# JoeMWatson/input-inference-for-control

Measured on AMD Instinct MI355X. Metric: i2c timestep-messages/sec (cell-iterations/s = B*T*EM-iters/s), pendulum T=200 B=4096 per GPU, higher is better.
Workload: dtype f64; 1 GPU; pendulum_known_quad cubature i2c (nx=2, nu=1, nz=4), T=200, B=4096 trajectories per GPU, global batch 4096, CubatureQuadrature(1,0,0), alpha0=100, tol=0; batch_per_gpu=4096, horizon=200, parallelism=batch-sharded x1, no collective in the EM loop, kernels=one lane per trajectory

## Files before the change

input-inference-for-control_amd/csrc/i2c_cell.hpp:

```cpp
#pragma once
#include <stdint.h>
#include <type_traits>
#include "../../include/i2c_hip.h"
#include "i2c_linalg.hpp"
#include "i2c_models.hpp"

namespace i2c {

template <typename R> struct Rule {
  R sf;
  R w0;
  R wi;
  R W;
  int unit;
  int gh_degree, gh_points;
  R gh_x[I2C_MAX_GH_DEGREE], gh_w[I2C_MAX_GH_DEGREE];
};

template <class M> struct PerTraj : M {};
template <class M> struct is_per_traj : std::false_type {};
template <class M> struct is_per_traj<PerTraj<M>> : std::true_type {};
template <typename R, bool PER_TRAJ> struct ParamsB {};
template <typename R> struct ParamsB<R, true> {
  const R* params_b;
// ... 1354 lines not shown
    for (int i = 0; i < NX; ++i) r.m3f[i] = in[(long)(O_MU3 + i) * B];
#pragma unroll
    for (int i = 0; i < sym(NX); ++i) r.S3f[i] = in[(long)(O_S3 + i) * B];
#pragma unroll
    for (int i = 0; i < NX * NX; ++i) r.Jx[i] = in[(long)(O_J + i) * B];
  };
  Row cur, nxt;
  load(t_hi - 1, cur);
  for (int t = t_hi - 1; t >= t_lo; --t) {
    load(t > t_lo ? t - 1 : t_lo, nxt);
    const R* mu1 = cur.mu1;
    const R* S1 = cur.S1;
    const R* m3f = cur.m3f;
    const R* Jx = cur.Jx;
    R S3n[sym(NX)];
#pragma unroll
    for (int i = 0; i < sym(NX); ++i) S3n[i] = Cc[i] - cur.S3f[i];
    R an[NX], Gn[NX * NX];
#pragma unroll
    for (int i = 0; i < NX; ++i) {
      R v = mu1[i];
#pragma unroll
      for (int k = 0; k < NX; ++k) v += Jx[i * NX + k] * (av[k] - m3f[k]);
      an[i] = v;
    }
#pragma unroll
    for (int i = 0; i < sym(NX); ++i) Cc[i] = S1[i];
    add_JDJt<NX, NX>(Jx, S3n, Cc);
#pragma unroll
    for (int i = 0; i < NX; ++i)
#pragma unroll
      for (int j = 0; j < NX; ++j) {
        R v = R(0);
#pragma unroll
        for (int k = 0; k < NX; ++k) v += Jx[i * NX + k] * G[k * NX + j];
        Gn[i * NX + j] = v;
      }
#pragma unroll
    for (int i = 0; i < NX; ++i) av[i] = an[i];
#pragma unroll
    for (int i = 0; i < NX * NX; ++i) G[i] = Gn[i];
    cur = nxt;
  }
  constexpr int EC = NX + NX * NX + sym(NX);
  R* out = a.comp + ((long)ch * EC) * B + b;
#pragma unroll
  for (int i = 0; i < NX; ++i) out[(long)i * B] = av[i];
#pragma unroll
  for (int i = 0; i < NX * NX; ++i) out[(long)(NX + i) * B] = G[i];
#pragma unroll
  for (int i = 0; i < sym(NX); ++i) out[(long)(NX + NX * NX + i) * B] = Cc[i];
}

template <class M, typename R, typename S_ = R, int GRID = 0>
I2C_HD inline void chunk_stitch_body(const Consts<M, R>& c, const ChunkArgs<R, S_>& a, const int b) {
  using C = Consts<M, R>;
  constexpr int NX = C::NX, D = C::D;
  constexpr int O_MU3 = D + sym(D), O_S3 = O_MU3 + NX, EC = NX + NX * NX + sym(NX);
  const long B = c.B;
  const S_* last = a.cell.fwd + ((long)(c.T - 1) * C::E_FWD) * B + b;
  R m3f[NX], S3f[sym(NX)], m[NX], S[sym(NX)];
#pragma unroll
  for (int i = 0; i < NX; ++i) m3f[i] = last[(long)(O_MU3 + i) * B];
#pragma unroll
  for (int i = 0; i < sym(NX); ++i) S3f[i] = last[(long)(O_S3 + i) * B];
  end_of_chain<M, R>(c, a.cell.temp, b, m3f, S3f, m, S, a.cell.status);
  terminal_obs_stats<M, R, GRID>(c, b, m, S, a.cell.term_stats, a.cell.status);
  R av[NX], G[NX * NX], Cc[sym(NX)], nav[NX], nG[NX * NX], nCc[sym(NX)];
  auto loadc = [&](int ch, R* la, R* lG, R* lC) {
    const R* cp = a.comp + ((long)(ch > 0 ? ch : 0) * EC) * B + b;
#pragma unroll
    for (int i = 0; i < NX; ++i) la[i] = cp[(long)i * B];
#pragma unroll
    for (int i = 0; i < NX * NX; ++i) lG[i] = cp[(long)(NX + i) * B];
#pragma unroll
    for (int i = 0; i < sym(NX); ++i) lC[i] = cp[(long)(NX + NX * NX + i) * B];
  };
  loadc(a.n_chunks - 1, av, G, Cc);
  for (int ch = a.n_chunks - 1; ch >= 0; --ch) {
    loadc(ch - 1, nav, nG, nCc);
    R* bo = a.bnd + ((long)ch * C::E_XM) * B + b;
#pragma unroll
    for (int i = 0; i < NX; ++i) bo[(long)i * B] = m[i];
#pragma unroll
    for (int i = 0; i < sym(NX); ++i) bo[(long)(NX + i) * B] = S[i];
    R mn[NX];
#pragma unroll
    for (int i = 0; i < NX; ++i) {
      R v = av[i];
#pragma unroll
      for (int k = 0; k < NX; ++k) v += G[i * NX + k] * m[k];
      mn[i] = v;
    }
    add_JDJt<NX, NX>(G, S, Cc);
#pragma unroll
    for (int i = 0; i < NX; ++i) m[i] = mn[i];
#pragma unroll
    for (int i = 0; i < sym(NX); ++i) S[i] = Cc[i];
#pragma unroll
    for (int i = 0; i < NX; ++i) av[i] = nav[i];
#pragma unroll
    for (int i = 0; i < NX * NX; ++i) G[i] = nG[i];
#pragma unroll
    for (int i = 0; i < sym(NX); ++i) Cc[i] = nCc[i];
  }
}

template <class M, typename R, typename S_ = R, bool LEANW = false, int GRID = 0>
I2C_HD inline void chunk_walk_body(const Consts<M, R>& c, const ChunkArgs<R, S_>& a, const int ch, const int b) {
  using C = Consts<M, R>;
  constexpr int NX = C::NX, NZ = C::NZ, D = C::D;
  constexpr int O_MU3 = D + sym(D), O_S3 = O_MU3 + NX, O_J = O_S3 + sym(NX);
  constexpr unsigned W = sizeof(S_);
  const unsigned long B = c.B;
  const unsigned bo = (unsigned)b * W, rb = (unsigned)(B * W);
  const int t_lo = ch * a.chunk_len, t_hi = (t_lo + a.chunk_len < c.T) ? t_lo + a.chunk_len : c.T;
  CellArgs<R, S_> ca = a.cell;
  if (LEANW) ca.xm = nullptr, ca.zpost = nullptr, ca.cell_stats = nullptr;
  const bool z_per_cell = LEANW ? false : c.z_per_cell != 0;
  R m3m[NX], S3m[sym(NX)];
  {
    const R* bi = a.bnd + ((long)ch * C::E_XM) * B + b;
#pragma unroll
    for (int i = 0; i < NX; ++i) m3m[i] = bi[(long)i * B];
#pragma unroll
    for (int i = 0; i < sym(NX); ++i) S3m[i] = bi[(long)(NX + i) * B];
  }
  constexpr bool DOUBLE_BUFFER = C::D <= 5;
  constexpr bool VOFF = I2C_WALK_VOFF && C::D <= 5;
  constexpr int NOFF = C::E_FWD > C::E_POST ? (C::E_FWD > C::E_ZPOST ? C::E_FWD : C::E_ZPOST) : (C::E_POST > C::E_ZPOST ? C::E_POST : C::E_ZPOST);
  unsigned voff[VOFF ? NOFF : 1];
  if (VOFF) {
#pragma unroll
    for (int e = 0; e < NOFF; ++e) voff[e] = bo + (unsigned)e * rb;
  }
  PolyTab<R> ptab;
  if (VOFF) poly_tab_init(ptab);
  const PolyTab<R>* const tab = VOFF ? &ptab : nullptr;
  R row[C::E_FWD], nxt[DOUBLE_BUFFER ? C::E_FWD : 1];
  if (DOUBLE_BUFFER) {
    const Window w = make_window(ca.fwd + (unsigned long)(t_hi - 1) * C::E_FWD * B, (unsigned long)C::E_FWD * rb);
#pragma unroll
    for (int e = 0; e < C::E_FWD; ++e) row[e] = (R)wld<S_>(w, VOFF ? 0u : e * rb, VOFF ? voff[e] : bo);
    if (LEANW) {
#pragma unroll
      for (int e = 0; e < C::E_FWD; ++e) row[e] = opaque(row[e]);
    }
  }
  R sum_m = R(0), sum_v = R(0);
  for (int t = t_hi - 1; t >= t_lo; --t) {
    {
      const int tp = DOUBLE_BUFFER ? (t > t_lo ? t - 1 : t_lo) : t;
      const Window w = make_window(ca.fwd + (unsigned long)tp * C::E_FWD * B, (unsigned long)C::E_FWD * rb);
#pragma unroll
      for (int e = 0; e < C::E_FWD; ++e)
        (DOUBLE_BUFFER ? nxt[DOUBLE_BUFFER ? e : 0] : row[e]) = (R)wld<S_>(w, VOFF ? 0u : e * rb, VOFF ? voff[e] : bo);
    }
    if (ca.xm) {
      S_* xo = const_cast<S_*>(ca.xm) + ((long)t * C::E_XM) * B + b;
#pragma unroll
      for (int i = 0; i < NX; ++i) xo[(long)i * B] = (S_)m3m[i];
#pragma unroll
      for (int i = 0; i < sym(NX); ++i) xo[(long)(NX + i) * B] = (S_)S3m[i];
    }
    R dm[NX], dS[sym(NX)], zt[NZ];
#pragma unroll
    for (int i = 0; i < NX; ++i) dm[i] = m3m[i] - row[O_MU3 + i];
#pragma unroll
    for (int i = 0; i < sym(NX); ++i) dS[i] = S3m[i] - row[O_S3 + i];
    if (VOFF && z_per_cell) {
      static_assert(NZ <= NOFF, "row offsets");
      const Window wz = make_window(ca.z + (unsigned long)c.row(t) * NZ * B, (unsigned long)NZ * B * sizeof(R));
#pragma unroll
      for (int k = 0; k < NZ; ++k) zt[k] = wld<R>(wz, 0u, voff[k] * (unsigned)(sizeof(R) / W));
    } else {
#pragma unroll
      for (int k = 0; k < NZ; ++k) zt[k] = z_per_cell ? ca.z[((long)c.row(t) * NZ + k) * B + b] : c.zg[k];
    }
    R* mu = row;
    R* S = row + D;
    R ctl[C::E_POST - D - sym(D)], mz[NZ], Sz[sym(NZ)], cm, cv;
    if (!cell_posterior<M, R, GRID>(c, b, zt, mu, S, row + O_J, dm, dS, ctl, mz, Sz, &cm, &cv, tab)) set_status(ca.status, b, 7, t);
    store_cell<M, R, S_>(c, ca, t, b, mu, S, ctl, mz, Sz, cm, cv, VOFF ? voff : nullptr);
    sum_m += cm;
    sum_v += cv;
#pragma unroll
    for (int i = 0; i < NX; ++i) m3m[i] = mu[i];
#pragma unroll
    for (int i = 0; i < sym(NX); ++i) S3m[i] = S[i];
    if (DOUBLE_BUFFER) {
#pragma unroll
      for (int e = 0; e < C::E_FWD; ++e) row[e] = nxt[DOUBLE_BUFFER ? e : 0];
    }
  }
  a.part[((long)ch * 2 + 0) * B + b] = sum_m;
  a.part[((long)ch * 2 + 1) * B + b] = sum_v;
}

template <typename R> struct MstepArgs {
  const R* term_stats;
  R* alpha;
  R* stats_out;
  int update;
};

template <class M, typename R>
I2C_HD inline void mstep_body(const Consts<M, R>& c, const MstepArgs<R>& a, const int b) {
  using C = Consts<M, R>;
  const long B = c.B;
  const R stat = a.term_stats[B + b], v = a.term_stats[2 * B + b];
  const R m = c.inference == I2C_INF_LINEARIZE ? a.term_stats[(long)(C::E_TERM - 1) * B + b] : stat;
  R tr = stat, sf = R(C::NZ) * R(c.T);
  if (C::NZT > 0 && c.has_Qf) {
    tr += a.term_stats[b];
    sf += R(C::NZT);
  }
  const R alpha_hat = tr / sf;
  const R alpha = a.alpha[b];
  R alpha_new = alpha;
  if (a.update) {
    if (c.tol >= R(0)) {
      const R ratio = alpha_hat / alpha;
      alpha_new = alpha_hat;
      if (ratio < c.tol) alpha_new = c.tol * alpha;
      if (ratio > R(2) - c.tol) alpha_new = (R(2) - c.tol) * alpha;
    }
    a.alpha[b] = alpha_new;
  }
  a.stats_out[b] = alpha_hat;
  a.stats_out[B + b] = alpha_new;
  a.stats_out[2 * B + b] = m;
  a.stats_out[3 * B + b] = v;
}

template <typename R> struct PropArgs {
  const R* post;
  R* prop;
  R* prop_stats;
  const R* x0;
  const R* sig_x0;
  const R* z;
  const uint8_t* ff;
  int32_t* status;
  const uint8_t* expert;
};

template <class M, typename R, int GRID = 0>
I2C_HD inline void propagate_body(const Consts<M, R>& c, const PropArgs<R>& a, const int b) {
  using C = Consts<M, R>;
  constexpr int NX = C::NX, NU = C::NU, NZ = C::NZ, D = C::D;
  const long B = c.B;
  const int T = c.T;
  const bool wr = grid_writer<GRID>();
  R mu_x[NX], sig_x[sym(NX)];
#pragma unroll
  for (int i = 0; i < NX; ++i) mu_x[i] = a.x0[i * B + b];
#pragma unroll
  for (int i = 0; i < sym(NX); ++i) sig_x[i] = a.sig_x0[i * B + b];
  constexpr bool PREFETCH = C::D <= 5;
  R pri[C::E_PRI];
  if (PREFETCH) {
#pragma unroll
    for (int e = 0; e < C::E_PRI; ++e) pri[e] = a.post[((long)c.row(0) * C::E_POST + e) * B + b];
  }
  unsigned ff_cur = a.ff[c.row(0)], ex_cur = a.expert ? (unsigned)a.expert[c.row(0)] : (unsigned)(c.use_expert != 0);
  ff_cur = opaque(ff_cur);
  ex_cur = opaque(ex_cur);
  if (PREFETCH) {
#pragma unroll
    for (int e = 0; e < C::E_PRI; ++e) pri[e] = opaque(pri[e]);
  }
#pragma unroll
  for (int i = 0; i < NX; ++i) mu_x[i] = opaque(mu_x[i]);
#pragma unroll
  for (int i = 0; i < sym(NX); ++i) sig_x[i] = opaque(sig_x[i]);
  constexpr bool ZPRE = PREFETCH && NZ <= NX * 4;
  R zt_cur[ZPRE ? NZ : 1];
  auto fetch_z = [&](const int row, R* zt) {
    const R* src = c.z_per_cell ? a.z + ((long)row * NZ) * B + b : a.x0 + b;
    const long st = c.z_per_cell ? B : 0;
#pragma unroll
    for (int k = 0; k < NZ; ++k) {
      const R v = src[(long)k * st];
      zt[k] = c.z_per_cell ? v : c.zg[k];
    }
// ... 446 lines not shown
```

input-inference-for-control_amd/csrc/i2c_impl.hpp:

```cpp
#pragma once
#include "i2c_entry.hpp"
#include "i2c_cell.hpp"
#include "i2c_group.hpp"
#include "i2c_wave.hpp"
#include "i2c_quad.hpp"
#include "i2c_grid.hpp"
#include "i2c_linearize.hpp"

#include <cmath>
#include <cstdlib>
#include <cstring>

namespace i2c {

constexpr int SWEEP_BLOCK = 64;
#ifndef I2C_LANE_BLOCK
#define I2C_LANE_BLOCK 64
#endif
constexpr int LANE_BLOCK = I2C_LANE_BLOCK;
constexpr int CELL_BLOCK = 256;

#ifdef I2C_HOST_SIM
#define I2C_KERNEL(BLOCK) static void
#define I2C_LANE_PARAMS const long lane_x_, const int lane_y_,
// ... 31 lines not shown
  return hipMemcpyAsync(dst, src, n, hipMemcpyDeviceToDevice, (hipStream_t)stream) == hipSuccess ? I2C_OK : I2C_ELAUNCH;
}
#endif

template <class M, typename R, bool LEAN, bool GRID = false, typename S = R>
I2C_KERNEL(LANE_BLOCK) k_forward(I2C_LANE_PARAMS const Consts<M, R> c, const FwdArgs<R, S> a, const int block) {
  const long b = I2C_LANE_X(block);
  if (b < c.B) forward_sweep_body<M, R, LEAN, GRID, S>(c, a, (int)b);
}
template <class M, typename R> I2C_KERNEL(LANE_BLOCK) k_forward_lin(I2C_LANE_PARAMS const Consts<M, R> c, const FwdArgs<R> a) {
  const long b = I2C_LANE_X(LANE_BLOCK);
  if (b < c.B) forward_lin_body<M, R>(c, a, (int)b);
}
template <class M, typename R> I2C_KERNEL(LANE_BLOCK) k_bwd_lin(I2C_LANE_PARAMS const Consts<M, R> c, const CellArgs<R> a) {
  const long b = I2C_LANE_X(LANE_BLOCK);
  if (b < c.B) backward_lin_body<M, R>(c, a, (int)b);
}
template <class M, typename R> I2C_KERNEL(LANE_BLOCK) k_riccati(I2C_LANE_PARAMS const Consts<M, R> c, const RiccatiArgs<R> a) {
  const long b = I2C_LANE_X(LANE_BLOCK);
  if (b < c.B) riccati_body<M, R>(c, a, (int)b);
}
template <class M, typename R, typename S = R>
I2C_KERNEL(LANE_BLOCK) k_scan(I2C_LANE_PARAMS const Consts<M, R> c, const ScanArgs<R, S> a) {
  const long b = I2C_LANE_X(LANE_BLOCK);
  if (b < c.B) backward_scan_body<M, R, S>(c, a, (int)b);
}
template <class M, typename R, typename S = R>
I2C_KERNEL(CELL_BLOCK) k_cell(I2C_LANE_PARAMS const Consts<M, R> c, const CellArgs<R, S> a) {
  const long b = I2C_LANE_X(CELL_BLOCK);
  if (b < c.B) backward_cell_body<M, R, S>(c, a, I2C_LANE_Y, (int)b);
}
template <class M, typename R, bool GRID = false, typename S = R, bool LEANW = false>
I2C_KERNEL(LANE_BLOCK) k_bwd_fused(I2C_LANE_PARAMS const Consts<M, R> c, const CellArgs<R, S> a) {
  const long b = I2C_LANE_X(LANE_BLOCK);
  if (b < c.B) backward_fused_body<M, R, GRID, S, LEANW>(c, a, (int)b);
}
template <class M, typename R, typename S = R>
I2C_KERNEL(LANE_BLOCK) k_chunk_compose(I2C_LANE_PARAMS const Consts<M, R> c, const ChunkArgs<R, S> a) {
  const long b = I2C_LANE_X(LANE_BLOCK);
  if (b < c.B) chunk_compose_body<M, R, S>(c, a, I2C_LANE_Y, (int)b);
}
template <class M, typename R, typename S = R, bool GRID = false>
I2C_KERNEL(LANE_BLOCK) k_chunk_stitch(I2C_LANE_PARAMS const Consts<M, R> c, const ChunkArgs<R, S> a) {
  const long b = I2C_LANE_X(LANE_BLOCK);
  if (b < c.B) chunk_stitch_body<M, R, S, GRID>(c, a, (int)b);
}
#ifndef I2C_WALK_LEAN
#define I2C_WALK_LEAN 1
#endif
template <class M, typename R, typename S = R, bool LEANW = false, bool GRID = false>
I2C_KERNEL(LANE_BLOCK) k_chunk_walk(I2C_LANE_PARAMS const Consts<M, R> c, const ChunkArgs<R, S> a) {
  const long b = I2C_LANE_X(LANE_BLOCK);
  if (b < c.B) chunk_walk_body<M, R, S, LEANW, GRID>(c, a, I2C_LANE_Y, (int)b);
}
template <class M, typename R> I2C_KERNEL(LANE_BLOCK) k_chunk_stitch_lin(I2C_LANE_PARAMS const Consts<M, R> c, const ChunkArgs<R, R> a) {
  const long b = I2C_LANE_X(LANE_BLOCK);
  if (b < c.B) chunk_stitch_lin_body<M, R>(c, a, (int)b);
}
template <class M, typename R> I2C_KERNEL(LANE_BLOCK) k_chunk_walk_lin(I2C_LANE_PARAMS const Consts<M, R> c, const ChunkArgs<R, R> a) {
  const long b = I2C_LANE_X(LANE_BLOCK);
  if (b < c.B) chunk_walk_lin_body<M, R>(c, a, I2C_LANE_Y, (int)b);
}
template <class M, typename R>
I2C_KERNEL(LANE_BLOCK) k_chunk_reduce_lin(I2C_LANE_PARAMS const Consts<M, R> c, const ChunkArgs<R, R> a, const MstepArgs<R> ms) {
  const long b = I2C_LANE_X(LANE_BLOCK);
  if (b < c.B) chunk_reduce_lin_body<M, R>(c, a, ms, (int)b);
}
template <class M, typename R> I2C_KERNEL(LANE_BLOCK) k_mstep(I2C_LANE_PARAMS const Consts<M, R> c, const MstepArgs<R> a) {
  const long b = I2C_LANE_X(LANE_BLOCK);
  if (b < c.B) mstep_body<M, R>(c, a, (int)b);
}
template <class M, typename R, bool GRID = false>
I2C_KERNEL(LANE_BLOCK) k_propagate(I2C_LANE_PARAMS const Consts<M, R> c, const PropArgs<R> a) {
  const long b = I2C_LANE_X(LANE_BLOCK);
  if (b < c.B) propagate_body<M, R, GRID>(c, a, (int)b);
}
template <class M, typename R, bool LEAN>
I2C_KERNEL(LANE_BLOCK) k_forward_propagate(I2C_LANE_PARAMS const Consts<M, R> c, const FwdArgs<R, R> af, const PropArgs<R> ap) {
  const long b = I2C_LANE_X(LANE_BLOCK);
  if (b >= c.B) return;
  if (I2C_LANE_Y == 0) forward_sweep_body<M, R, LEAN, false, R>(c, af, (int)b);
  else propagate_body<M, R, false>(c, ap, (int)b);
}
template <class M, typename R> struct ZetaArg {
  R v[sym(M::NY)];
};
template <class M, typename R>
I2C_KERNEL(LANE_BLOCK) k_ckf(I2C_LANE_PARAMS const Consts<M, R> c, const ZetaArg<M, R> z, const CkfArgs<R> a) {
  const long b = I2C_LANE_X(LANE_BLOCK);
  if (b < c.B) ckf_filter_body<M, R>(c, z.v, a, (int)b);
}
template <class M, typename R> I2C_KERNEL(CELL_BLOCK) k_mpc_shift(I2C_LANE_PARAMS const Consts<M, R> c, const ShiftArgs<R> a) {
  const long b = I2C_LANE_X(CELL_BLOCK);
  if (b < c.B) mpc_shift_body<M, R>(c, a, (int)b);
}
template <class M> I2C_KERNEL(CELL_BLOCK) k_to_feedback(I2C_LANE_PARAMS uint8_t* ff, const int t0, const int n, const int T) {
  const long i = I2C_LANE_X(CELL_BLOCK);
  if (i < n) ff[(t0 + (int)i) % T] = 0;
}
template <class M, typename R> I2C_KERNEL(LANE_BLOCK) k_rollout(I2C_LANE_PARAMS const Consts<M, R> c, const RolloutArgs<R> a) {
  const long n = I2C_LANE_X(LANE_BLOCK);
  if (n < (long)a.n_rollouts * c.B) rollout_body<M, R>(c, a, (int)n);
}
template <class M, typename R>
I2C_KERNEL(LANE_BLOCK) k_plant_step(I2C_LANE_PARAMS const Consts<M, R> c, const PlantNoise<M, R> nz, const PlantArgs<R> a) {
  const long b = I2C_LANE_X(LANE_BLOCK);
// ... 6 lines not shown
                          const R m, const R v) {
  a.term_stats[(long)c.B + b] = m;
  a.term_stats[2 * (long)c.B + b] = v;
  if (ms.alpha) {
    Consts<M, R> cm = c;
    cm.T = T_mstep;
    mstep_body<M, R>(cm, ms, b);
  }
}
#ifdef I2C_HOST_SIM
template <class M, typename R, class CA>
static int launch_reduce(const Consts<M, R>& c, const CA& a, const MstepArgs<R>& ms, const int T_mstep, void*) {
  for (int b = 0; b < c.B; ++b) {
    R m = R(0), v = R(0);
    for (int q = 0; q < REDUCE_PARTS; ++q) {
      R pm, pv;
      reduce_partial<M, R>(c, a.cell_stats, b, q, REDUCE_PARTS, &pm, &pv);
      m += pm;
      v += pv;
    }
    reduce_finish<M, R>(c, a, ms, T_mstep, b, m, v);
  }
  return I2C_OK;
}
#else
template <class M, typename R, class CA>
__global__ __launch_bounds__(SWEEP_BLOCK* REDUCE_PARTS) void k_reduce(const Consts<M, R> c, const CA a,
                                                                      const MstepArgs<R> ms, const int T_mstep) {
  __shared__ R sm[REDUCE_PARTS][SWEEP_BLOCK], sv[REDUCE_PARTS][SWEEP_BLOCK];
  const int b = blockIdx.x * SWEEP_BLOCK + threadIdx.x;
  R m = R(0), v = R(0);
  if (b < c.B) reduce_partial<M, R>(c, a.cell_stats, b, threadIdx.y, REDUCE_PARTS, &m, &v);
  sm[threadIdx.y][threadIdx.x] = m;
  sv[threadIdx.y][threadIdx.x] = v;
  __syncthreads();
  if (threadIdx.y == 0 && b < c.B) {
    m = sm[0][threadIdx.x];
    v = sv[0][threadIdx.x];
#pragma unroll
    for (int q = 1; q < REDUCE_PARTS; ++q) {
      m += sm[q][threadIdx.x];
      v += sv[q][threadIdx.x];
    }
    reduce_finish<M, R>(c, a, ms, T_mstep, b, m, v);
  }
}
template <class M, typename R, class CA>
static int launch_reduce(const Consts<M, R>& c, const CA& a, const MstepArgs<R>& ms, const int T_mstep, void* stream) {
  hipLaunchKernelGGL((k_reduce<M, R, CA>), dim3((c.B + SWEEP_BLOCK - 1) / SWEEP_BLOCK), dim3(SWEEP_BLOCK, REDUCE_PARTS), 0,
                     (hipStream_t)stream, c, a, ms, T_mstep);
  return hipGetLastError() == hipSuccess ? I2C_OK : I2C_ELAUNCH;
}
#endif


template <typename R> static bool unit_rule(const Rule<R>& r) { return r.unit && r.w0 == R(0); }
template <class M, typename R> static bool unit_rule(const Consts<M, R>& c) { return unit_rule(c.rule_xu) && unit_rule(c.rule_x); }

#ifdef I2C_HOST_SIM
template <typename R, class Body>
static void sim_teams(const int team, const long n_teams, const int n_rows, const bool rows_on_team, const size_t lds, const Body& body) {
  for (int y0 = 0; y0 < (rows_on_team ? 1 : n_rows); ++y0)
    for (long i = 0; i < n_teams; ++i) {
      std::vector<R> sh(lds, R(0)), xch(128, R(0));
      HostBarrier bar(team);
      std::vector<std::thread> lanes;
      for (int l = 0; l < team; ++l)
        lanes.emplace_back([&, l] {
          for (int y = y0; y < (rows_on_team ? n_rows : y0 + 1); ++y) body(i, y, l, lds ? sh.data() : (R*)nullptr, &bar, xch.data());
        });
      for (auto& th : lanes) th.join();
    }
}
#else
template <class M, typename R> __device__ __forceinline__ const Consts<M, R>* kernarg_consts() {
  return (const Consts<M, R>*)__builtin_amdgcn_kernarg_segment_ptr();
}
template <class M, typename R> __device__ __forceinline__ const R* kernarg_zeta() {
  constexpr size_t zoff = (sizeof(Consts<M, R>) + alignof(ZetaArg<M, R>) - 1) / alignof(ZetaArg<M, R>) * alignof(ZetaArg<M, R>);
  return ((const ZetaArg<M, R>*)((const char*)__builtin_amdgcn_kernarg_segment_ptr() + zoff))->v;
}
__device__ __forceinline__ long xcd_first_traj(const unsigned i) {
  const unsigned x = i & 7u, r = (i >> 3) & 3u, g = i >> 5;
  return 16L * (g * 8u + x) + 4 * r;
}
static unsigned xcd_blocks(const long B) { return (unsigned)((B + 127) / 128) * 32u; }
#endif

enum { GK_FORWARD = 0, GK_BACKWARD = 1, GK_PROPAGATE = 2, GK_CKF = 3 };
template <int KIND, class M, typename R, int G, bool FULLW, class KC, class A>
I2C_FN void group_body(const Consts<M, R>& c, const KC& kc, const A& a, const int b, const Grp<R, G>& g) {
  if constexpr (KIND == GK_FORWARD) forward_group_body<M, R, G, FULLW>(c, kc, a, b, g);
  if constexpr (KIND == GK_BACKWARD) backward_group_body<M, R, G, FULLW>(c, kc, a, b, g);
  if constexpr (KIND == GK_PROPAGATE) propagate_group_body<M, R, G, FULLW>(c, kc, a, b, g);
  if constexpr (KIND == GK_CKF) ckf_group_body<M, R, G>(c, kc, a, b, g);
}
#ifndef I2C_HOST_SIM
template <int KIND, class M, typename R, int G, bool FULLW, class A>
__global__ __launch_bounds__(SWEEP_BLOCK) void k_group(const Consts<M, R> c, const ZetaArg<M, R> zeta, const int has_zeta, const A a) {
  __shared__ GConst<M, R> kc;
  __shared__ R sh[(SWEEP_BLOCK / G) * Grp<R, G>::SIZE];
  gconst_fill<M, R>(kc, kernarg_consts<M, R>(), has_zeta ? kernarg_zeta<M, R>() : (const R*)nullptr, (int)threadIdx.x, SWEEP_BLOCK);
  __syncthreads();
  const long lane = (long)blockIdx.x * SWEEP_BLOCK + threadIdx.x;
  const long b = lane / G;
  if (b >= c.B) return;
// ... 383 lines not shown
  C c;
  std::memset(&c, 0, sizeof(c));
  c.B = p->B;
  c.T = p->T;
  c.t0 = p->t0;
  c.has_Qf = p->has_Qf && M::NZT > 0;
  c.has_x_terminal = p->has_x_terminal;
  c.z_per_cell = p->z_per_cell && p->z != nullptr;
  c.use_expert = use_expert;
  c.terminal_cell = p->terminal_cell;
  c.inference = p->inference;
  c.post_tm = (p->post_layout == 1 && M::WAVE) ? 1 : 0;
  auto is_diag = [](const double* W, int n) {
    for (int i = 0; i < n; ++i)
      for (int j = 0; j < i; ++j)
        if (W[i * (i + 1) / 2 + j] != 0.0) return 0;
    return 1;
  };
  c.qr_diag = is_diag(p->QR, C::NZ);
  c.qf_diag = is_diag(p->Qf, C::NZT);
  c.rule_xu = make_rule<R>(p, C::D);
  c.rule_x = make_rule<R>(p, C::NX);
  c.dtemp = (R)p->dtemp;
  c.tol = (R)tol;
  for (int i = 0; i < sym(C::NX); ++i) c.sig_eta[i] = (R)p->sig_eta[i];
  for (int i = 0; i < sym(C::NX); ++i) c.sig_eta_w[i] = c.rule_xu.W * c.sig_eta[i];
  for (int i = 0; i < sym(C::NZ); ++i) c.sig_xi0[i] = (R)p->sig_xi0[i];
  for (int i = 0; i < sym(C::NZ); ++i) c.QR[i] = (R)p->QR[i];
  for (int i = 0; i < sym(C::NZT); ++i) c.sig_xiT0[i] = (R)p->sig_xiT0[i];
  for (int i = 0; i < sym(C::NZT); ++i) c.Qf[i] = (R)p->Qf[i];
  for (int i = 0; i < C::NZ; ++i) c.zg[i] = (R)p->zg[i];
  for (int i = 0; i < C::NZT; ++i) c.zg_term[i] = (R)p->zg_term[i];
  for (int i = 0; i < C::NX; ++i) c.mu_x_term[i] = (R)p->mu_x_term[i];
  for (int i = 0; i < sym(C::NX); ++i) c.sig_x_term[i] = (R)p->sig_x_term[i];
  for (int i = 0; i < M::NP; ++i) c.params[i] = (R)p->model_params[i];
  if constexpr (is_per_traj<M>::value) c.params_b = (const R*)p->model_params_b;
  return c;
}

static void chunk_geometry(int B, int T, int* n_chunks, int* chunk_len) {
  static const int forced = [] {
    const char* e = getenv("I2C_CHUNKS");
    return e ? atoi(e) : 0;
  }();
  int nc = (65536 + B - 1) / B;
  if (nc > 32) nc = 32;
  if (nc > T / 4) nc = T / 4;
  if (forced > 0) nc = forced < T ? forced : T;
  if (nc < 1) nc = 1;
  const int len = (T + nc - 1) / nc;
  *chunk_len = len;
  *n_chunks = (T + len - 1) / len;
}
template <class M> struct ChunkWork {
  size_t bnd, part, total;
  ChunkWork(const int B, const int n_chunks) {
    constexpr int NX = M::NX;
    const size_t n = (size_t)n_chunks * (size_t)B;
    bnd = n * (NX + NX * NX + sym(NX));
    part = bnd + n * (NX + sym(NX));
    total = part + n * 3;
  }
};
template <class M> static size_t workspace_elems(int B, int T) {
  int nc, len;
  chunk_geometry(B, T, &nc, &len);
  return ChunkWork<M>(B, nc).total;
}
template <class M, typename R, typename S> static ChunkArgs<R, S> chunk_args(const I2cProblem* p, const CellArgs<R, S>& a) {
  ChunkArgs<R, S> ch{a, (R*)p->work, nullptr, nullptr, 0, 0};
  chunk_geometry(p->B, p->T, &ch.n_chunks, &ch.chunk_len);
  const ChunkWork<M> w(p->B, ch.n_chunks);
  ch.bnd = ch.comp + w.bnd;
  ch.part = ch.comp + w.part;
  return ch;
}

#define I2C_MODEL_CONST(name, MEMBER, DEFAULT)                                                                      \
  template <class M, class = void> struct name : std::integral_constant<int, (DEFAULT)> {};                         \
  template <class M> struct name<M, std::void_t<decltype(M::MEMBER)>> : std::integral_constant<int, M::MEMBER> {};
I2C_MODEL_CONST(bwd_fused_min_b, BWD_FUSED_MIN_B, I2C_BWD_FUSED_MIN_B)
I2C_MODEL_CONST(quad_backward_min_b, QUAD_BACKWARD8_MIN_B, 0)
I2C_MODEL_CONST(quad_backward_max_b, QUAD_BACKWARD8_MAX_B, -1)
I2C_MODEL_CONST(quad_chunk_walk_min_b, QUAD_CHUNK_WALK_MIN_B, 0)
I2C_MODEL_CONST(quad_chunk_walk_max_b, QUAD_CHUNK_WALK_MAX_B, -1)
I2C_MODEL_CONST(quad_chunk_passes_min_b, QUAD_CHUNK_PASSES_MIN_B, 0)
I2C_MODEL_CONST(quad_chunk_passes_max_b, QUAD_CHUNK_PASSES_MAX_B, -1)
I2C_MODEL_CONST(quad_chunk_stitch_max_b, QUAD_CHUNK_STITCH_MAX_B, -1)
#undef I2C_MODEL_CONST


struct Plan {
  int forward, backward, propagate, filter;
  int schedule;
  int walker;
  int compose, stitch;
  int rule;
  bool fwd_tm;
  bool fusable;
};

template <class M, typename R, typename S = R> struct Impl {
  using C = Consts<M, R>;
  static constexpr bool MIXED = sizeof(S) != sizeof(R);
  static constexpr int G = M::GROUP;
  static constexpr bool HAS_GROUP = G > 0 && sizeof(R) == 8 && !MIXED;
// ... 197 lines not shown

  static Plan resolve(const I2cProblem* p) {
    const Rule<R> rule_xu = make_rule<R>(p, C::D), rule_x = make_rule<R>(p, C::NX);
    const bool unit_xu = unit_rule(rule_xu), unit = unit_xu && unit_rule(rule_x);
    const Request req = request(p->group_lanes, p->inference);
    Plan pl;
    pl.rule = p->inference;
    pl.forward = forward_family(p, req, unit);
    pl.backward = backward_family(p, req, unit);
    pl.propagate = propagate_family(p, req, unit_xu || p->inference == I2C_INF_LINEARIZE);
    pl.filter = filter_family(p, req == REQ_GRID ? request(p->group_lanes, I2C_INF_CUBATURE) : req);
    pl.schedule = backward_schedule(p, req, pl.backward);
    const bool chunked = pl.schedule == I2C_BWD_CHUNKED;
    pl.walker = chunked ? pl.backward : I2C_ENOTSUP;
    pl.compose = pl.stitch = pl.schedule < 0 ? pl.schedule : I2C_ENOTSUP;
    if (chunked && p->inference == I2C_INF_CUBATURE) {
      pl.compose = quad_compose(p, req, unit) ? I2C_FAMILY_QUAD : I2C_FAMILY_LANE;
      pl.stitch = (pl.compose == I2C_FAMILY_QUAD || quad_stitch_alone(p, req, unit)) ? I2C_FAMILY_QUAD : I2C_FAMILY_LANE;
    }
    pl.fwd_tm = !MIXED && pl.forward == I2C_FAMILY_QUAD && ((M::WAVE && pl.backward == I2C_FAMILY_WAVE) || (HAS_QUAD_BACKWARD && pl.backward == I2C_FAMILY_QUAD));
    pl.fusable = LANE && C::D <= 5 && p->inference == I2C_INF_CUBATURE && pl.forward == I2C_FAMILY_LANE && pl.propagate == I2C_FAMILY_LANE &&
                 rule_xu.unit && rule_x.unit && !(p->z_per_cell && p->z) && !p->alpha_cell && p->t0 == 0;
    return pl;
  }
  static int plan(const I2cProblem* p) { return resolve(p).schedule; }
  static int family_of(const I2cProblem* p, const int sweep) {
    const Plan pl = resolve(p);
    const int of_sweep[] = {pl.forward, pl.backward, pl.propagate, pl.filter, pl.compose, pl.stitch};
    return of_sweep[sweep];
  }
  static int schedule_with(const Plan& pl, const bool workspace) {
    if (pl.schedule != I2C_BWD_CHUNKED || workspace) return pl.schedule;
    return (pl.rule == I2C_INF_CUBATURE && pl.walker != I2C_FAMILY_QUAD) ? I2C_BWD_TWO_PASS : I2C_BWD_FUSED;
  }

  static I2cProblem with_unit_rule(const I2cProblem* p) {
    I2cProblem q = *p;
    q.quad_alpha = 1.0, q.quad_beta = 0.0, q.quad_kappa = 0.0;
    return q;
  }
  static C forward_consts(const I2cProblem* p) { return make_consts<M, R>(p, 0.0, p->inference == I2C_INF_LINEARIZE ? p->expert_controller : 0); }
  static C propagate_consts(const I2cProblem* p, const int use_expert) {
    if (p->inference != I2C_INF_LINEARIZE) return make_consts<M, R>(p, 0.0, use_expert);
    const I2cProblem q = with_unit_rule(p);
    return make_consts<M, R>(&q, 0.0, use_expert);
  }
  static C filter_consts(const I2cProblem* p) {
    I2cProblem q = with_unit_rule(p);
    q.inference = I2C_INF_CUBATURE;
    return make_consts<M, R>(&q, 0.0, 0);
  }

  static int run_forward(const I2cProblem* p, const Plan& pl, const C& c, const void* prior, void* fwd, void* prior_out, int32_t* status,
                         void* stream) {
    if (pl.forward < 0) return pl.forward;
    const FwdArgs<R, S> a{(const S*)prior, (S*)fwd, (S*)prior_out, (const R*)p->x0, (const R*)p->sig_x0,
                          (const R*)p->z,  (const R*)p->alpha, (const R*)p->alpha_cell, p->feedforward, status, p->expert};
    if (pl.forward == I2C_FAMILY_WAVE) {
      if constexpr (HAS_WAVE) return launch_wave<WK_FORWARD, M, R, S>(c, a, stream);
    }
    if (pl.forward == I2C_FAMILY_QUAD) {
      if constexpr (HAS_QUAD) {
        C cq = c;
        cq.fwd_tm = pl.fwd_tm;
        return launch_quad_forward<M, R, S>(cq, a, stream);
      }
    }
    if (pl.forward == I2C_FAMILY_GROUP) {
      if constexpr (HAS_GROUP) return launch_group<GK_FORWARD, M, R, G>(c, nullptr, a, stream);
    }
    if (pl.forward == I2C_FAMILY_GRID) {
      if constexpr (HAS_GRID) return launch_grid<GRK_FORWARD, M, R>(c, a, stream);
    }
    if constexpr (LANE) {
      if constexpr (!MIXED) {
        if (pl.rule == I2C_INF_LINEARIZE) return launch(k_forward_lin<M, R>, p->B, 1, LANE_BLOCK, stream, c, a);
        if (pl.rule == I2C_INF_GAUSS_HERMITE) return launch(k_forward<M, R, false, true>, p->B, 1, LANE_BLOCK, stream, c, a, LANE_BLOCK);
      }
#ifdef I2C_HOST_SIM
      const int lanes = LANE_BLOCK;
#else
      const int lanes = sweep_lanes();
#endif
      const bool lean = c.rule_xu.unit && c.rule_x.unit && !c.z_per_cell && !a.alpha_cell && !a.prior_out && c.t0 == 0;
      if (lean) return launch(k_forward<M, R, true, false, S>, p->B, 1, lanes, stream, c, a, lanes);
      return launch(k_forward<M, R, false, false, S>, p->B, 1, lanes, stream, c, a, lanes);
    }
    return I2C_ENOTSUP;
  }
  static int forward(const I2cProblem* p, const void* prior, void* fwd, void* prior_out, int32_t* status, void* stream) {
    return run_forward(p, resolve(p), forward_consts(p), prior, fwd, prior_out, status, stream);
  }

  struct MstepFuse {
    double tol;
    int update;
    void* stats_out;
    bool done;
  };
  static const R* terminal_alpha(const I2cProblem* p, const C& c) {
    return p->alpha_cell ? (const R*)p->alpha_cell + (long)c.row(p->T - 1) * (long)p->B : (const R*)p->alpha;
  }
  static int run_backward(const I2cProblem* p, const Plan& pl, const C& c, const void* fwd, void* xm, void* post, void* zpost, void* cell_stats,
                          void* term_stats, int32_t* status, void* stream, MstepFuse* fuse) {
    if (pl.backward < 0) return pl.backward;
    if (pl.schedule < 0) return pl.schedule;
    const MstepArgs<R> ms{(const R*)term_stats, fuse ? (R*)p->alpha : nullptr, fuse ? (R*)fuse->stats_out : nullptr, fuse ? fuse->update : 0};
    const CellArgs<R, S> a{(const S*)fwd,  (const S*)xm,   (const R*)p->z, (S*)post, (S*)zpost,
                           (R*)cell_stats, (R*)term_stats, (R*)p->temp,    status,   terminal_alpha(p, c)};
    const int mode = schedule_with(pl, p->work != nullptr);
    int rc = I2C_ENOTSUP;
    if (pl.backward == I2C_FAMILY_WAVE) {
      if constexpr (HAS_WAVE) {
        if (mode != I2C_BWD_TWO_PASS || !a.xm || !a.cell_stats) return launch_wave<WK_BACKWARD, M, R, S>(c, a, stream);
        rc = launch_wave<WK_SCAN, M, R, S>(c, a, stream);
        if (rc == I2C_OK) rc = launch_wave<WK_CELL, M, R, S>(c, a, stream);
        if (rc == I2C_OK) rc = launch_reduce<M, R>(c, a, ms, p->T, stream);
        if (fuse) fuse->done = true;
      }
      return rc;
    }
    if (pl.backward == I2C_FAMILY_QUAD) {
      if constexpr (HAS_QUAD_BACKWARD) {
        if constexpr (QUAD8) {
          if (mode == I2C_BWD_CHUNKED) return backward_chunked(p, pl, c, a, ms, fuse, stream);
        }
        return launch_quad_backward<M, R, S>(c, a, stream);
      }
    }
    if (pl.backward == I2C_FAMILY_GROUP) {
      if constexpr (HAS_GROUP) return launch_group<GK_BACKWARD, M, R, G>(c, nullptr, a, stream);
    }
    if (pl.backward == I2C_FAMILY_GRID) {
      if constexpr (HAS_GRID) return launch_grid<GRK_BACKWARD, M, R>(c, a, stream);
    }
    if constexpr (LANE) {
      if (mode == I2C_BWD_CHUNKED) return backward_chunked(p, pl, c, a, ms, fuse, stream);
      if (mode == I2C_BWD_FUSED) {
        if constexpr (!MIXED) {
          if (pl.rule == I2C_INF_LINEARIZE) return launch(k_bwd_lin<M, R>, p->B, 1, LANE_BLOCK, stream, c, a);
          if (pl.rule == I2C_INF_GAUSS_HERMITE) return launch(k_bwd_fused<M, R, true>, p->B, 1, LANE_BLOCK, stream, c, a);
        }
        const bool lean = I2C_WALK_LEAN && !a.xm && !a.zpost && !a.cell_stats && !c.z_per_cell;
        return lean ? launch(k_bwd_fused<M, R, false, S, true>, p->B, 1, LANE_BLOCK, stream, c, a)
                    : launch(k_bwd_fused<M, R, false, S>, p->B, 1, LANE_BLOCK, stream, c, a);
      }
      if (!a.xm || !a.cell_stats) return I2C_EINVAL;
      const ScanArgs<R, S> sc{a.fwd, const_cast<S*>(a.xm), (R*)p->temp, a.status};
      rc = launch(k_scan<M, R, S>, p->B, 1, LANE_BLOCK, stream, c, sc);
      if (rc == I2C_OK) rc = launch(k_cell<M, R, S>, p->B, p->T, CELL_BLOCK, stream, c, a);
      if (rc == I2C_OK) rc = launch_reduce<M, R>(c, a, ms, p->T, stream);
      if (fuse) fuse->done = true;
    }
    return rc;
  }
  static int backward_chunked(const I2cProblem* p, const Plan& pl, const C& c, const CellArgs<R, S>& a, const MstepArgs<R>& ms, MstepFuse* fuse,
                              void* stream) {
    int rc = I2C_ENOTSUP;
    if constexpr (LANE) {
      const ChunkArgs<R, S> ch = chunk_args<M>(p, a);
      const long B = p->B;
      const int nc = ch.n_chunks;
      const bool lin = !MIXED && pl.rule == I2C_INF_LINEARIZE, gh = !MIXED && pl.rule == I2C_INF_GAUSS_HERMITE;
      if (fuse) fuse->done = true;
      if (pl.compose == I2C_FAMILY_QUAD) {
        if constexpr (QUAD8) rc = launch_quad_chunk_compose<M, R, S>(c, ch, stream);
      } else {
        rc = launch(k_chunk_compose<M, R, S>, B, nc, LANE_BLOCK, stream, c, ch);
      }
      if (rc != I2C_OK) return rc;
      rc = I2C_ENOTSUP;
      if (pl.stitch == I2C_FAMILY_QUAD) {
        if constexpr (QUAD8) rc = launch_quad_chunk_stitch<M, R, S>(c, ch, stream);
      } else if (lin || gh) {
        if constexpr (!MIXED)
          rc = lin ? launch(k_chunk_stitch_lin<M, R>, B, 1, LANE_BLOCK, stream, c, ch) : launch(k_chunk_stitch<M, R, R, true>, B, 1, LANE_BLOCK, stream, c, ch);
      } else {
        rc = launch(k_chunk_stitch<M, R, S>, B, 1, LANE_BLOCK, stream, c, ch);
      }
      if (rc != I2C_OK) return rc;
      rc = I2C_ENOTSUP;
      if (pl.walker == I2C_FAMILY_QUAD) {
        if constexpr (QUAD8) rc = launch_quad_chunk_walk<M, R, S>(c, ch, stream);
      } else if (lin || gh) {
        if constexpr (!MIXED)
          rc = lin ? launch(k_chunk_walk_lin<M, R>, B, nc, LANE_BLOCK, stream, c, ch) : launch(k_chunk_walk<M, R, R, false, true>, B, nc, LANE_BLOCK, stream, c, ch);
      } else {
        const bool lean = I2C_WALK_LEAN && !a.xm && !a.zpost && !a.cell_stats && !c.z_per_cell;
        rc = lean ? launch(k_chunk_walk<M, R, S, true>, B, nc, LANE_BLOCK, stream, c, ch) : launch(k_chunk_walk<M, R, S>, B, nc, LANE_BLOCK, stream, c, ch);
      }
      if (rc != I2C_OK) return rc;
      if (lin) {
        if constexpr (!MIXED) rc = launch(k_chunk_reduce_lin<M, R>, B, 1, LANE_BLOCK, stream, c, ch, ms);
      } else {
        C cr = c;
        cr.T = nc;
        CellArgs<R, S> ared = a;
        ared.cell_stats = ch.part;
        rc = launch_reduce<M, R>(cr, ared, ms, p->T, stream);
      }
    }
    return rc;
  }
  static int backward(const I2cProblem* p, const void* fwd, void* xm, void* post, void* zpost, void* cell_stats,
                      void* term_stats, int32_t* status, void* stream) {
    return run_backward(p, resolve(p), make_consts<M, R>(p, 0.0, 0), fwd, xm, post, zpost, cell_stats, term_stats, status, stream, nullptr);
  }

  static int riccati(const I2cProblem* p, const void* prior_out, const void* fwd, const void* xm, void* post, void* ric,
                     int32_t* status, void* stream) {
    if constexpr (MIXED) return I2C_ENOTSUP;
    if constexpr (LANE) {
      if (!lane_request(p->group_lanes)) return I2C_ENOTSUP;
      const C c = make_consts<M, R>(p, 0.0, 0);
      RiccatiArgs<R> a{(const R*)prior_out, (const R*)fwd, (const R*)xm, (const R*)p->z, (const R*)p->alpha,
                       (R*)post,            (R*)ric,       status};
      return launch(k_riccati<M, R>, p->B, 1, LANE_BLOCK, stream, c, a);
    }
    return I2C_ENOTSUP;
  }

  static int run_mstep(const I2cProblem* p, const C& c, const void* term_stats, int update, void* stats_out, void* stream) {
    MstepArgs<R> a{(const R*)term_stats, (R*)p->alpha, (R*)stats_out, update};
    return launch(k_mstep<M, R>, p->B, 1, LANE_BLOCK, stream, c, a);
  }
  static int mstep(const I2cProblem* p, const void* term_stats, double tol, int update, void* stats_out, void* stream) {
    return run_mstep(p, make_consts<M, R>(p, tol, 0), term_stats, update, stats_out, stream);
  }

  static int to_feedback(const I2cProblem* p, int tau, void* stream) {
    const int n = tau + 1 < p->T ? tau + 1 : p->T;
    return launch(k_to_feedback<M>, n, 1, CELL_BLOCK, stream, const_cast<uint8_t*>(p->feedforward), p->t0, n, p->T);
  }

  static int learn(const I2cProblem* p, void* post, void* fwd, void* xm, void* zpost, void* cell_stats,
                   void* term_stats, double tol, int tau, int n_iters, void* stats_hist, int32_t* status,
                   void* stream) {
    const Plan pl = resolve(p);
    const C cf = forward_consts(p), cb = make_consts<M, R>(p, tol, 0);
    for (int it = 0; it < n_iters; ++it) {
      void* stats = (R*)stats_hist + (size_t)it * 4 * p->B;
      MstepFuse fuse{tol, 1, stats, false};
      int rc = run_forward(p, pl, cf, post, fwd, nullptr, status, stream);
      if (rc == I2C_OK) rc = run_backward(p, pl, cb, fwd, xm, post, zpost, cell_stats, term_stats, status, stream, &fuse);
      if (rc == I2C_OK && !fuse.done) rc = run_mstep(p, cb, term_stats, 1, stats, stream);
      if (rc == I2C_OK && tau > 0 && it == 0) rc = to_feedback(p, tau, stream);
      if (rc != I2C_OK) return rc;
    }
    return I2C_OK;
  }

  static int learn_propagate(const I2cProblem* p, void* post, void* fwd, void* xm, void* zpost, void* cell_stats, void* term_stats,
                             void* prop, void* prop_hist, double tol, int tau, int n_iters, void* stats_hist, int use_expert,
                             int overlap, int32_t* status, void* stream) {
    if constexpr (MIXED) return I2C_ENOTSUP;
    const Plan pl = resolve(p);
    const C cf = forward_consts(p), cb = make_consts<M, R>(p, tol, 0), cp = propagate_consts(p, use_expert);
    auto prop_row = [&](int it) { return (void*)((R*)prop_hist + (size_t)it * 3 * p->B); };
    int pending = -1;
    for (int it = 0; it < n_iters; ++it) {
      int rc = I2C_OK;
      bool fused = false;
      if constexpr (LANE && C::D <= 5) {
        if (overlap && pl.fusable && pending >= 0) {
          FwdArgs<R> af{(const R*)post, (R*)fwd, nullptr, (const R*)p->x0, (const R*)p->sig_x0, (const R*)p->z, (const R*)p->alpha,
                        (const R*)p->alpha_cell, p->feedforward, status, p->expert};
          PropArgs<R> ap{(const R*)post, (R*)prop, (R*)prop_row(pending), (const R*)p->x0, (const R*)p->sig_x0,
                         (const R*)p->z, p->feedforward, status, p->expert};
          rc = launch(k_forward_propagate<M, R, true>, p->B, 2, LANE_BLOCK, stream, cp, af, ap);
          fused = true;
          pending = -1;
        }
      }
      if (!fused) {
        if (pending >= 0) {
          rc = run_propagate(p, pl, cp, post, prop, prop_row(pending), status, stream);
          pending = -1;
          if (rc != I2C_OK) return rc;
        }
        rc = run_forward(p, pl, cf, post, fwd, nullptr, status, stream);
      }
      if (rc != I2C_OK) return rc;
      void* stats = (R*)stats_hist + (size_t)it * 4 * p->B;
      MstepFuse fuse{tol, 1, stats, false};
      rc = run_backward(p, pl, cb, fwd, xm, post, zpost, cell_stats, term_stats, status, stream, &fuse);
      if (rc != I2C_OK) return rc;
      if (it == 0) {
        rc = run_propagate(p, pl, cp, post, prop, prop_row(0), status, stream);
        if (rc != I2C_OK) return rc;
      } else {
        pending = it;
      }
      if (!fuse.done) rc = run_mstep(p, cb, term_stats, 1, stats, stream);
      if (rc == I2C_OK && tau > 0 && it == 0) rc = to_feedback(p, tau, stream);
      if (rc != I2C_OK) return rc;
    }
    if (pending >= 0) return run_propagate(p, pl, cp, post, prop, prop_row(pending), status, stream);
// ... 138 lines not shown
```

Baseline: 2.342 billion timestep-messages/s.

## Self-stitch chunk walkers and defer reduce+M-step into next forward kernel

Removes the serial chunk-stitch kernel: each chunk walker now recomputes its own boundary state by applying the downstream chunk composites directly, batching composite loads for latency hiding. It also defers the partial-sum reduction and M-step into the next iteration's forward kernel, which saves two kernel launches per EM iteration. In exchange each walker does redundant composite work that grows with the number of chunks, and the M-step timing is shifted into the forward pass.

```diff
diff --git a/input-inference-for-control_amd/csrc/i2c_cell.hpp b/input-inference-for-control_amd/csrc/i2c_cell.hpp
--- a/input-inference-for-control_amd/csrc/i2c_cell.hpp
+++ b/input-inference-for-control_amd/csrc/i2c_cell.hpp
@@ -1430,6 +1430,22 @@
   for (int i = 0; i < sym(NX); ++i) out[(long)(NX + NX * NX + i) * B] = Cc[i];
 }
 
+template <int NX, typename R> I2C_FN void apply_composite(const R* av, const R* G, R* Cc, R* m, R* S) {
+  R mn[NX];
+#pragma unroll
+  for (int i = 0; i < NX; ++i) {
+    R v = av[i];
+#pragma unroll
+    for (int k = 0; k < NX; ++k) v += G[i * NX + k] * m[k];
+    mn[i] = v;
+  }
+  add_JDJt<NX, NX>(G, S, Cc);
+#pragma unroll
+  for (int i = 0; i < NX; ++i) m[i] = mn[i];
+#pragma unroll
+  for (int i = 0; i < sym(NX); ++i) S[i] = Cc[i];
+}
+
 template <class M, typename R, typename S_ = R, int GRID = 0>
 I2C_HD inline void chunk_stitch_body(const Consts<M, R>& c, const ChunkArgs<R, S_>& a, const int b) {
   using C = Consts<M, R>;
@@ -1462,19 +1478,7 @@
     for (int i = 0; i < NX; ++i) bo[(long)i * B] = m[i];
 #pragma unroll
     for (int i = 0; i < sym(NX); ++i) bo[(long)(NX + i) * B] = S[i];
-    R mn[NX];
-#pragma unroll
-    for (int i = 0; i < NX; ++i) {
-      R v = av[i];
-#pragma unroll
-      for (int k = 0; k < NX; ++k) v += G[i * NX + k] * m[k];
-      mn[i] = v;
-    }
-    add_JDJt<NX, NX>(G, S, Cc);
-#pragma unroll
-    for (int i = 0; i < NX; ++i) m[i] = mn[i];
-#pragma unroll
-    for (int i = 0; i < sym(NX); ++i) S[i] = Cc[i];
+    apply_composite<NX, R>(av, G, Cc, m, S);
 #pragma unroll
     for (int i = 0; i < NX; ++i) av[i] = nav[i];
 #pragma unroll
@@ -1484,7 +1488,33 @@
   }
 }
 
-template <class M, typename R, typename S_ = R, bool LEANW = false, int GRID = 0>
+template <class M, typename R, typename S_>
+I2C_FN void chunk_boundary_state(const Consts<M, R>& c, const ChunkArgs<R, S_>& a, const int ch, const int b, R* m, R* S) {
+  using C = Consts<M, R>;
+  constexpr int NX = C::NX, D = C::D;
+  constexpr int O_MU3 = D + sym(D), O_S3 = O_MU3 + NX, EC = NX + NX * NX + sym(NX);
+  constexpr int DEPTH = NX <= 2 ? 8 : 4;
+  const long B = c.B;
+  const S_* last = a.cell.fwd + ((long)(c.T - 1) * C::E_FWD) * B + b;
+#pragma unroll
+  for (int i = 0; i < NX; ++i) m[i] = last[(long)(O_MU3 + i) * B];
+#pragma unroll
+  for (int i = 0; i < sym(NX); ++i) S[i] = last[(long)(O_S3 + i) * B];
+  for (int hi = a.n_chunks - 1; hi > ch; hi -= DEPTH) {
+    R comp[DEPTH][EC];
+#pragma unroll
+    for (int k = 0; k < DEPTH; ++k) {
+      const R* cp = a.comp + ((long)(hi - k > ch ? hi - k : ch + 1) * EC) * B + b;
+#pragma unroll
+      for (int i = 0; i < EC; ++i) comp[k][i] = cp[(long)i * B];
+    }
+#pragma unroll
+    for (int k = 0; k < DEPTH; ++k)
+      if (hi - k > ch) apply_composite<NX, R>(comp[k], comp[k] + NX, comp[k] + NX + NX * NX, m, S);
+  }
+}
+
+template <class M, typename R, typename S_ = R, bool LEANW = false, int GRID = 0, bool SELF = false>
 I2C_HD inline void chunk_walk_body(const Consts<M, R>& c, const ChunkArgs<R, S_>& a, const int ch, const int b) {
   using C = Consts<M, R>;
   constexpr int NX = C::NX, NZ = C::NZ, D = C::D;
@@ -1497,7 +1527,7 @@
   if (LEANW) ca.xm = nullptr, ca.zpost = nullptr, ca.cell_stats = nullptr;
   const bool z_per_cell = LEANW ? false : c.z_per_cell != 0;
   R m3m[NX], S3m[sym(NX)];
-  {
+  if (!SELF) {
     const R* bi = a.bnd + ((long)ch * C::E_XM) * B + b;
 #pragma unroll
     for (int i = 0; i < NX; ++i) m3m[i] = bi[(long)i * B];
@@ -1520,6 +1550,11 @@
     const Window w = make_window(ca.fwd + (unsigned long)(t_hi - 1) * C::E_FWD * B, (unsigned long)C::E_FWD * rb);
 #pragma unroll
     for (int e = 0; e < C::E_FWD; ++e) row[e] = (R)wld<S_>(w, VOFF ? 0u : e * rb, VOFF ? voff[e] : bo);
+    if (SELF) {
+      static_assert(!SELF || (GRID == 0 && DOUBLE_BUFFER), "the self-stitching walker: sigma-point rule, d <= 5");
+      chunk_boundary_state<M, R, S_>(c, a, ch, b, m3m, S3m);
+      if (ch == a.n_chunks - 1) terminal_obs_stats<M, R, GRID>(c, b, m3m, S3m, ca.term_stats, ca.status);
+    }
     if (LEANW) {
 #pragma unroll
       for (int e = 0; e < C::E_FWD; ++e) row[e] = opaque(row[e]);
@@ -1583,18 +1618,16 @@
 };
 
 template <class M, typename R>
-I2C_HD inline void mstep_body(const Consts<M, R>& c, const MstepArgs<R>& a, const int b) {
+I2C_FN void mstep_update(const Consts<M, R>& c, const MstepArgs<R>& a, const int b, const R trT, const R stat, const R v, const R m,
+                         const R alpha) {
   using C = Consts<M, R>;
   const long B = c.B;
-  const R stat = a.term_stats[B + b], v = a.term_stats[2 * B + b];
-  const R m = c.inference == I2C_INF_LINEARIZE ? a.term_stats[(long)(C::E_TERM - 1) * B + b] : stat;
   R tr = stat, sf = R(C::NZ) * R(c.T);
   if (C::NZT > 0 && c.has_Qf) {
-    tr += a.term_stats[b];
+    tr += trT;
     sf += R(C::NZT);
   }
   const R alpha_hat = tr / sf;
-  const R alpha = a.alpha[b];
   R alpha_new = alpha;
   if (a.update) {
     if (c.tol >= R(0)) {
@@ -1609,6 +1642,15 @@
   a.stats_out[B + b] = alpha_new;
   a.stats_out[2 * B + b] = m;
   a.stats_out[3 * B + b] = v;
+}
+template <class M, typename R>
+I2C_HD inline void mstep_body(const Consts<M, R>& c, const MstepArgs<R>& a, const int b) {
+  using C = Consts<M, R>;
+  const long B = c.B;
+  const R stat = a.term_stats[B + b], v = a.term_stats[2 * B + b];
+  const R m = c.inference == I2C_INF_LINEARIZE ? a.term_stats[(long)(C::E_TERM - 1) * B + b] : stat;
+  const R trT = (C::NZT > 0 && c.has_Qf) ? a.term_stats[b] : R(0);
+  mstep_update<M, R>(c, a, b, trT, stat, v, m, a.alpha[b]);
 }
 
 template <typename R> struct PropArgs {
diff --git a/input-inference-for-control_amd/csrc/i2c_impl.hpp b/input-inference-for-control_amd/csrc/i2c_impl.hpp
--- a/input-inference-for-control_amd/csrc/i2c_impl.hpp
+++ b/input-inference-for-control_amd/csrc/i2c_impl.hpp
@@ -107,6 +107,11 @@
 I2C_KERNEL(LANE_BLOCK) k_chunk_walk(I2C_LANE_PARAMS const Consts<M, R> c, const ChunkArgs<R, S> a) {
   const long b = I2C_LANE_X(LANE_BLOCK);
   if (b < c.B) chunk_walk_body<M, R, S, LEANW, GRID>(c, a, I2C_LANE_Y, (int)b);
+}
+template <class M, typename R, typename S = R, bool LEANW = false>
+I2C_KERNEL(LANE_BLOCK) k_chunk_walk_self(I2C_LANE_PARAMS const Consts<M, R> c, const ChunkArgs<R, S> a) {
+  const long b = I2C_LANE_X(LANE_BLOCK);
+  if (b < c.B) chunk_walk_body<M, R, S, LEANW, 0, true>(c, a, I2C_LANE_Y, (int)b);
 }
 template <class M, typename R> I2C_KERNEL(LANE_BLOCK) k_chunk_stitch_lin(I2C_LANE_PARAMS const Consts<M, R> c, const ChunkArgs<R, R> a) {
   const long b = I2C_LANE_X(LANE_BLOCK);
@@ -219,6 +224,59 @@
   return hipGetLastError() == hipSuccess ? I2C_OK : I2C_ELAUNCH;
 }
 #endif
+
+template <typename R> struct PendingMstep {
+  const R* part;
+  R* term_stats;
+  MstepArgs<R> ms;
+  int n_chunks;
+  R tol;
+};
+template <class M, typename R> I2C_FN void finish_pending_mstep(const Consts<M, R>& c, const PendingMstep<R>& pm, const int b) {
+  using C = Consts<M, R>;
+  constexpr int P = REDUCE_PARTS;
+  const long B = c.B;
+  const int nc = pm.n_chunks;
+  const R alpha = pm.ms.alpha[b];
+  const R trT = (C::NZT > 0 && c.has_Qf) ? pm.term_stats[b] : R(0);
+  R sm[P], sv[P];
+#pragma unroll
+  for (int q = 0; q < P; ++q) sm[q] = sv[q] = R(0);
+  for (int t0 = 0; t0 < nc; t0 += 2 * P) {
+    R pm_t[2 * P], pv_t[2 * P];
+#pragma unroll
+    for (int i = 0; i < 2 * P; ++i) {
+      const long t = t0 + i < nc ? t0 + i : nc - 1;
+      pm_t[i] = pm.part[(t * 2 + 0) * B + b];
+      pv_t[i] = pm.part[(t * 2 + 1) * B + b];
+    }
+#pragma unroll
+    for (int i = 0; i < 2 * P; ++i) {
+      const bool in = t0 + i < nc;
+      sm[i % P] += in ? pm_t[i] : R(0);
+      sv[i % P] += in ? pv_t[i] : R(0);
+    }
+  }
+  R m = R(0), v = R(0);
+#pragma unroll
+  for (int q = 0; q < P; ++q) {
+    m += sm[q];
+    v += sv[q];
+  }
+  pm.term_stats[B + b] = m;
+  pm.term_stats[2 * B + b] = v;
+  Consts<M, R> cm = c;
+  cm.tol = pm.tol;
+  mstep_update<M, R>(cm, pm.ms, b, trT, m, v, m, alpha);
+}
+template <class M, typename R, bool LEAN, typename S = R>
+I2C_KERNEL(LANE_BLOCK) k_forward_mstep(I2C_LANE_PARAMS const Consts<M, R> c, const FwdArgs<R, S> a, const int block, const PendingMstep<R> pm) {
+  const long b = I2C_LANE_X(block);
+  if (b < c.B) {
+    finish_pending_mstep<M, R>(c, pm, (int)b);
+    forward_sweep_body<M, R, LEAN, 0, S>(c, a, (int)b);
+  }
+}
 
 
 template <typename R> static bool unit_rule(const Rule<R>& r) { return r.unit && r.w0 == R(0); }
@@ -708,6 +766,10 @@
   *chunk_len = len;
   *n_chunks = (T + len - 1) / len;
 }
+static bool chunk_four_passes() {
+  const char* e = getenv("I2C_CHUNK_PASSES");
+  return e && atoi(e) == 4;
+}
 template <class M> struct ChunkWork {
   size_t bnd, part, total;
   ChunkWork(const int B, const int n_chunks) {
@@ -1011,8 +1073,9 @@
   }
 
   static int run_forward(const I2cProblem* p, const Plan& pl, const C& c, const void* prior, void* fwd, void* prior_out, int32_t* status,
-                         void* stream) {
+                         void* stream, const PendingMstep<R>* pend = nullptr) {
     if (pl.forward < 0) return pl.forward;
+    if (pend && !defers_mstep(pl)) return I2C_EINVAL;
     const FwdArgs<R, S> a{(const S*)prior, (S*)fwd, (S*)prior_out, (const R*)p->x0, (const R*)p->sig_x0,
                           (const R*)p->z,  (const R*)p->alpha, (const R*)p->alpha_cell, p->feedforward, status, p->expert};
     if (pl.forward == I2C_FAMILY_WAVE) {
@@ -1042,6 +1105,10 @@
       const int lanes = sweep_lanes();
 #endif
       const bool lean = c.rule_xu.unit && c.rule_x.unit && !c.z_per_cell && !a.alpha_cell && !a.prior_out && c.t0 == 0;
+      if constexpr (SELF_STITCH) {
+        if (pend) return lean ? launch(k_forward_mstep<M, R, true, S>, p->B, 1, lanes, stream, c, a, lanes, *pend)
+                              : launch(k_forward_mstep<M, R, false, S>, p->B, 1, lanes, stream, c, a, lanes, *pend);
+      }
       if (lean) return launch(k_forward<M, R, true, false, S>, p->B, 1, lanes, stream, c, a, lanes);
       return launch(k_forward<M, R, false, false, S>, p->B, 1, lanes, stream, c, a, lanes);
     }
@@ -1056,7 +1123,16 @@
     int update;
     void* stats_out;
     bool done;
+    bool defer;
+    bool deferred;
+    PendingMstep<R> pending;
   };
+  static constexpr bool SELF_STITCH = LANE && C::D <= 5;
+  static bool self_stitches(const Plan& pl, const C& c) {
+    return SELF_STITCH && pl.rule == I2C_INF_CUBATURE && pl.stitch == I2C_FAMILY_LANE && pl.walker == I2C_FAMILY_LANE && !c.has_x_terminal &&
+           !chunk_four_passes();
+  }
+  static bool defers_mstep(const Plan& pl) { return SELF_STITCH && pl.rule == I2C_INF_CUBATURE && pl.forward == I2C_FAMILY_LANE; }
   static const R* terminal_alpha(const I2cProblem* p, const C& c) {
     return p->alpha_cell ? (const R*)p->alpha_cell + (long)c.row(p->T - 1) * (long)p->B : (const R*)p->alpha;
   }
@@ -1121,6 +1197,7 @@
       const long B = p->B;
       const int nc = ch.n_chunks;
       const bool lin = !MIXED && pl.rule == I2C_INF_LINEARIZE, gh = !MIXED && pl.rule == I2C_INF_GAUSS_HERMITE;
+      const bool self = self_stitches(pl, c);
       if (fuse) fuse->done = true;
       if (pl.compose == I2C_FAMILY_QUAD) {
         if constexpr (QUAD8) rc = launch_quad_chunk_compose<M, R, S>(c, ch, stream);
@@ -1134,8 +1211,10 @@
       } else if (lin || gh) {
         if constexpr (!MIXED)
           rc = lin ? launch(k_chunk_stitch_lin<M, R>, B, 1, LANE_BLOCK, stream, c, ch) : launch(k_chunk_stitch<M, R, R, true>, B, 1, LANE_BLOCK, stream, c, ch);
+      } else if (!self) {
+        rc = launch(k_chunk_stitch<M, R, S>, B, 1, LANE_BLOCK, stream, c, ch);
       } else {
-        rc = launch(k_chunk_stitch<M, R, S>, B, 1, LANE_BLOCK, stream, c, ch);
+        rc = I2C_OK;
       }
       if (rc != I2C_OK) return rc;
       rc = I2C_ENOTSUP;
@@ -1146,11 +1225,19 @@
           rc = lin ? launch(k_chunk_walk_lin<M, R>, B, nc, LANE_BLOCK, stream, c, ch) : launch(k_chunk_walk<M, R, R, false, true>, B, nc, LANE_BLOCK, stream, c, ch);
       } else {
         const bool lean = I2C_WALK_LEAN && !a.xm && !a.zpost && !a.cell_stats && !c.z_per_cell;
-        rc = lean ? launch(k_chunk_walk<M, R, S, true>, B, nc, LANE_BLOCK, stream, c, ch) : launch(k_chunk_walk<M, R, S>, B, nc, LANE_BLOCK, stream, c, ch);
+        if constexpr (SELF_STITCH) {
+          if (self)
+            rc = lean ? launch(k_chunk_walk_self<M, R, S, true>, B, nc, LANE_BLOCK, stream, c, ch)
+                      : launch(k_chunk_walk_self<M, R, S>, B, nc, LANE_BLOCK, stream, c, ch);
+        }
+        if (!self) rc = lean ? launch(k_chunk_walk<M, R, S, true>, B, nc, LANE_BLOCK, stream, c, ch) : launch(k_chunk_walk<M, R, S>, B, nc, LANE_BLOCK, stream, c, ch);
       }
       if (rc != I2C_OK) return rc;
       if (lin) {
         if constexpr (!MIXED) rc = launch(k_chunk_reduce_lin<M, R>, B, 1, LANE_BLOCK, stream, c, ch, ms);
+      } else if (self && fuse && fuse->defer) {
+        fuse->deferred = true;
+        fuse->pending = PendingMstep<R>{ch.part, a.term_stats, ms, nc, c.tol};
       } else {
         C cr = c;
         cr.T = nc;
@@ -1197,11 +1284,15 @@
                    void* stream) {
     const Plan pl = resolve(p);
     const C cf = forward_consts(p), cb = make_consts<M, R>(p, tol, 0);
+    PendingMstep<R> pend{};
+    bool have_pend = false;
     for (int it = 0; it < n_iters; ++it) {
       void* stats = (R*)stats_hist + (size_t)it * 4 * p->B;
-      MstepFuse fuse{tol, 1, stats, false};
-      int rc = run_forward(p, pl, cf, post, fwd, nullptr, status, stream);
+      MstepFuse fuse{tol, 1, stats, false, it + 1 < n_iters && defers_mstep(pl), false, {}};
+      int rc = run_forward(p, pl, cf, post, fwd, nullptr, status, stream, have_pend ? &pend : nullptr);
+      have_pend = false;
       if (rc == I2C_OK) rc = run_backward(p, pl, cb, fwd, xm, post, zpost, cell_stats, term_stats, status, stream, &fuse);
+      if (rc == I2C_OK && fuse.deferred) pend = fuse.pending, have_pend = true;
       if (rc == I2C_OK && !fuse.done) rc = run_mstep(p, cb, term_stats, 1, stats, stream);
       if (rc == I2C_OK && tau > 0 && it == 0) rc = to_feedback(p, tau, stream);
       if (rc != I2C_OK) return rc;
```

Result: faster. 2.378 billion timestep-messages/s (median of 6 runs) (+1.5%).
